# choderalab/pymbar

Measured on AMD Instinct MI355X. Metric: mbar_adaptive_iterations_per_sec, higher is better.
Workload: dtype f64

## Files before the change

### pymbar_amd/csrc/mbar_device.h

```cpp
#ifndef MBAR_DEVICE_H
#define MBAR_DEVICE_H
#include "mbar_internal.h"

#include <hip/hip_ext.h>
#include <math.h>
#include <type_traits>

namespace mbar {

typedef double v4d __attribute__((ext_vector_type(4)));

template <int CTRL>
__device__ __forceinline__ double dpp_move(double x) {
    int lo = __double2loint(x), hi = __double2hiint(x);
    lo = __builtin_amdgcn_update_dpp(0, lo, CTRL, 0xF, 0xF, true);
    hi = __builtin_amdgcn_update_dpp(0, hi, CTRL, 0xF, 0xF, true);
    return __hiloint2double(hi, lo);
}
__device__ __forceinline__ double row16_max(double x) {
    x = fmax(x, dpp_move<0xB1>(x));
    x = fmax(x, dpp_move<0x4E>(x));
    x = fmax(x, dpp_move<0x141>(x));
    x = fmax(x, dpp_move<0x140>(x));
    return x;
}
template <int N>
__device__ __forceinline__ double row16_bcast(double x) {
    double r;
    asm("v_mov_b64_dpp %0, %1 row_newbcast:%2 row_mask:0xf bank_mask:0xf" : "=v"(r) : "v"(x), "n"(N));
    return r;
}
__device__ __forceinline__ double row16_sum(double x) {
    x += dpp_move<0xB1>(x);
    x += dpp_move<0x4E>(x);
    x += dpp_move<0x141>(x);
    x += dpp_move<0x140>(x);
    return x;
}
template <int M>
__device__ __forceinline__ double lane_xor(double x) {
    if constexpr (M >= 16) {
        return __shfl_xor(x, M);
    } else if constexpr (M == 8) {
        return dpp_move<0x128>(x);
    } else if constexpr (M == 4) {
        int lo = __double2loint(x), hi = __double2hiint(x);
        int tl = __builtin_amdgcn_update_dpp(lo, lo, 0x104, 0xF, 0x5, false);
        tl = __builtin_amdgcn_update_dpp(tl, lo, 0x114, 0xF, 0xA, false);
        int th = __builtin_amdgcn_update_dpp(hi, hi, 0x104, 0xF, 0x5, false);
        th = __builtin_amdgcn_update_dpp(th, hi, 0x114, 0xF, 0xA, false);
        return __hiloint2double(th, tl);
    } else if constexpr (M == 2) {
        return dpp_move<0x4E>(x);
    } else {
        return dpp_move<0xB1>(x);
    }
}
__device__ __forceinline__ double wave_sum(double x) {
#pragma unroll
    for (int m = 32; m >= 1; m >>= 1) x += __shfl_xor(x, m);
    return x;
}
__device__ __forceinline__ double wave_max(double x) {
#pragma unroll
    for (int m = 32; m >= 1; m >>= 1) x = fmax(x, __shfl_xor(x, m));
    return x;
}
__device__ __forceinline__ double block256_sum(double v, double* red ) {
    v = wave_sum(v);
    __syncthreads();
    if ((threadIdx.x & 63) == 0) red[threadIdx.x >> 6] = v;
    __syncthreads();
    return (red[0] + red[1]) + (red[2] + red[3]);
}
__device__ __forceinline__ double block256_max(double v, double* red ) {
    v = wave_max(v);
    __syncthreads();
    if ((threadIdx.x & 63) == 0) red[threadIdx.x >> 6] = v;
    __syncthreads();
    return fmax(fmax(red[0], red[1]), fmax(red[2], red[3]));
}

#include "exp2_table.inc"
#include "log_table.inc"
constexpr double LOG2E = 0x1.71547652b82fep+0, LN2 = 0x1.62e42fefa39efp-1;
constexpr double EXP2_S = (double)(1 << EXP2_BITS);
constexpr double LOG2E_S = EXP2_S * LOG2E, LN2_OVER_S = LN2 / EXP2_S;
constexpr double EXP2_CLAMP = -1100.0 * EXP2_S;
constexpr int EXP2_TABLE_BYTES = (1 << EXP2_BITS) * 8;
constexpr int LOG_TABLE_BYTES = 256 * 8;
constexpr int EXP_TABLE_BYTES = EXP2_TABLE_BYTES + LOG_TABLE_BYTES;
constexpr int EXP_TABLE_DMA_PER_WAVE = (EXP_TABLE_BYTES / 1024 + 7) / 8;
typedef __attribute__((address_space(3))) const double lds_cdouble;
__device__ __forceinline__ void exp_table_init(char* smem) {
    if ((uint32_t)(uintptr_t)(__attribute__((address_space(3))) char*)smem != 0u) __builtin_trap();
    for (int i = threadIdx.x; i < (1 << EXP2_BITS); i += blockDim.x) reinterpret_cast<double*>(smem)[i] = EXP2_TABLE[i];
    for (int i = threadIdx.x; i < 256; i += blockDim.x)
        reinterpret_cast<double*>(smem + EXP2_TABLE_BYTES)[i] = LOG_TABLE[i];
}
__device__ __forceinline__ void exp_table_init_dma(char* smem) {
    if ((uint32_t)(uintptr_t)(__attribute__((address_space(3))) char*)smem != 0u) __builtin_trap();
    const int lane = threadIdx.x & 63;
    const int wave = __builtin_amdgcn_readfirstlane(threadIdx.x >> 6), nwv = blockDim.x >> 6;
    constexpr int NCH = EXP_TABLE_BYTES / 1024, NCH_EXP = EXP2_TABLE_BYTES / 1024;
    const int per_wave = (NCH + nwv - 1) / nwv;
    for (int i = 0; i < per_wave; ++i) {
        const int c = (wave + i * nwv) % NCH;
        const char* src = c < NCH_EXP ? reinterpret_cast<const char*>(EXP2_TABLE) + c * 1024
                                      : reinterpret_cast<const char*>(LOG_TABLE) + (c - NCH_EXP) * 1024;
        __builtin_amdgcn_global_load_lds((const __attribute__((address_space(1))) void*)(src + lane * 16),
                                         (__attribute__((address_space(3))) void*)(smem + c * 1024), 16, 0, 0);
    }
}
__device__ __forceinline__ double exp2_table_at(int si) {
    return *(lds_cdouble*)(uintptr_t)(uint32_t)((si << 3) & (EXP2_TABLE_BYTES - 8));
}
__device__ __forceinline__ double exp2_poly(double z) {
    double p = EXP2_POLY[EXP2_DEG];
#pragma unroll
    for (int k = EXP2_DEG - 1; k >= 0; --k) p = fma(p, z, EXP2_POLY[k]);
    return p;
}
__device__ __forceinline__ double exp2s_fast(double ts) {
    const double t = fmax(ts, EXP2_CLAMP);
    const double s = __builtin_rint(t);
    const double z = t - s;
    const int si = (int)s;
    const double T = exp2_table_at(si);
    return ldexp(T * exp2_poly(z), si >> EXP2_BITS);
}
typedef double v2d __attribute__((ext_vector_type(2)));
__device__ __forceinline__ double log_pos(double s) {
    const double m = __builtin_amdgcn_frexp_mant(s);
    const double ed = (double)__builtin_amdgcn_frexp_exp(s);
    const uint32_t off = (uint32_t)(__double2hiint(m) >> 9) & 0x7f0u;
    const v2d tc = *(__attribute__((address_space(3))) const v2d*)(uintptr_t)(uint32_t)(EXP2_TABLE_BYTES + off);
    const double r = fma(m, tc.x, -1.0);
    double q = -1.0 / 6.0;
    q = fma(q, r, 0.2);
    q = fma(q, r, -0.25);
    q = fma(q, r, 1.0 / 3.0);
    q = fma(q, r, -0.5);
    q = fma(q, r, 1.0);
    return fma(ed, LN2, tc.y) + q * r;
}
template <int N, bool CLAMP = true>
__device__ __forceinline__ void exp2s_batch(double (&x)[N]) {
    double T[N];
    int q[N];
#pragma unroll
    for (int i = 0; i < N; ++i) {
        const double t = CLAMP ? fmax(x[i], EXP2_CLAMP) : x[i];
        const double s = __builtin_rint(t);
        x[i] = t - s;
        const int si = (int)s;
        q[i] = si >> EXP2_BITS;
        T[i] = exp2_table_at(si);
    }
    __builtin_amdgcn_sched_barrier(0);
#pragma unroll
    for (int i = 0; i < N; ++i) x[i] = exp2_poly(x[i]);
    __builtin_amdgcn_sched_barrier(0);
#pragma unroll
    for (int i = 0; i < N; ++i) x[i] = ldexp(T[i] * x[i], q[i]);
}
template <int N>
__device__ __forceinline__ void exp2s_batch2(double (&x0)[N], double (&x1)[N]) {
    double T0[N], T1[N];
    int q0[N], q1[N];
#pragma unroll
    for (int i = 0; i < N; ++i) {
        const double t0 = fmax(x0[i], EXP2_CLAMP), t1 = fmax(x1[i], EXP2_CLAMP);
        const double s0 = __builtin_rint(t0), s1 = __builtin_rint(t1);
        x0[i] = t0 - s0;
        x1[i] = t1 - s1;
        const int i0 = (int)s0, i1 = (int)s1;
        q0[i] = i0 >> EXP2_BITS;
        q1[i] = i1 >> EXP2_BITS;
        T0[i] = exp2_table_at(i0);
        T1[i] = exp2_table_at(i1);
    }
    __builtin_amdgcn_sched_barrier(0);
#pragma unroll
    for (int i = 0; i < N; ++i) {
        x0[i] = exp2_poly(x0[i]);
        x1[i] = exp2_poly(x1[i]);
    }
    __builtin_amdgcn_sched_barrier(0);
#pragma unroll
    for (int i = 0; i < N; ++i) {
        x0[i] = ldexp(T0[i] * x0[i], q0[i]);
        x1[i] = ldexp(T1[i] * x1[i], q1[i]);
    }
}
constexpr double EXP2N_POLY[4] = {1.0, -0x1.62e42fefa3028p-12, 0x1.ebfbdf9648000p-25, -0x1.c69cea0000000p-38};
template <int N, bool CLAMP>
__device__ __forceinline__ void exp2s_neg_batch(double (&w)[N]) {
    double T[N];
    int q[N];
#pragma unroll
    for (int i = 0; i < N; ++i) {
        const double t = CLAMP ? fmin(w[i], 2.0e9) : w[i];
        const int ni = (int)(-t);
        w[i] = __builtin_amdgcn_fract(t);
        q[i] = ni >> EXP2_BITS;
        T[i] = exp2_table_at(ni);
    }
    __builtin_amdgcn_sched_barrier(0);
#pragma unroll
    for (int i = 0; i < N; ++i) {
        double p = EXP2N_POLY[3];
        p = fma(p, w[i], EXP2N_POLY[2]);
        p = fma(p, w[i], EXP2N_POLY[1]);
        w[i] = fma(p, w[i], EXP2N_POLY[0]);
    }
    __builtin_amdgcn_sched_barrier(0);
#pragma unroll
    for (int i = 0; i < N; ++i) w[i] = ldexp(T[i] * w[i], q[i]);
}
template <int N, bool CLAMP>
__device__ __forceinline__ void exp2s_neg_batch2(double (&w0)[N], double (&w1)[N]) {
    double T0[N], T1[N];
    int q0[N], q1[N];
#pragma unroll
    for (int i = 0; i < N; ++i) {
        const double t0 = CLAMP ? fmin(w0[i], 2.0e9) : w0[i], t1 = CLAMP ? fmin(w1[i], 2.0e9) : w1[i];
        const int n0 = (int)(-t0), n1 = (int)(-t1);
        w0[i] = __builtin_amdgcn_fract(t0);
        w1[i] = __builtin_amdgcn_fract(t1);
        q0[i] = n0 >> EXP2_BITS;
        q1[i] = n1 >> EXP2_BITS;
        T0[i] = exp2_table_at(n0);
        T1[i] = exp2_table_at(n1);
    }
    __builtin_amdgcn_sched_barrier(0);
#pragma unroll
    for (int i = 0; i < N; ++i) {
        double p0 = EXP2N_POLY[3], p1 = EXP2N_POLY[3];
        p0 = fma(p0, w0[i], EXP2N_POLY[2]);
        p1 = fma(p1, w1[i], EXP2N_POLY[2]);
        p0 = fma(p0, w0[i], EXP2N_POLY[1]);
        p1 = fma(p1, w1[i], EXP2N_POLY[1]);
        w0[i] = fma(p0, w0[i], EXP2N_POLY[0]);
        w1[i] = fma(p1, w1[i], EXP2N_POLY[0]);
    }
    __builtin_amdgcn_sched_barrier(0);
#pragma unroll
    for (int i = 0; i < N; ++i) {
        w0[i] = ldexp(T0[i] * w0[i], q0[i]);
        w1[i] = ldexp(T1[i] * w1[i], q1[i]);
    }
}
__device__ __forceinline__ double recip_fast(double s) {
    double r = __builtin_amdgcn_rcp(s);
    r = fma(fma(-s, r, 1.0), r, r);
    r = fma(fma(-s, r, 1.0), r, r);
    return r;
}

template <int NB>
__device__ __forceinline__ double tree_max(const double (&x)[NB]) {
    double t[NB];
#pragma unroll
    for (int i = 0; i < NB; ++i) t[i] = x[i];
#pragma unroll
    for (int n = NB; n > 1; n -= n / 2) {
#pragma unroll
        for (int i = 0; i < n / 2; ++i) t[i] = fmax(t[i], t[n - 1 - i]);
    }
    return t[0];
}
template <int NB>
__device__ __forceinline__ double tree_sum(const double (&x)[NB]) {
    double t[NB];
#pragma unroll
    for (int i = 0; i < NB; ++i) t[i] = x[i];
#pragma unroll
    for (int n = NB; n > 1; n -= n / 2) {
#pragma unroll
        for (int i = 0; i < n / 2; ++i) t[i] += t[n - 1 - i];
    }
    return t[0];
}
template <int NB>
__device__ __forceinline__ double dot_sum(const double (&x)[NB], const double (&c)[NB]) {
    if constexpr (NB == 1) {
        return x[0] * c[0];
    } else {
        double e = x[0] * c[0], o = x[1] * c[1];
#pragma unroll
        for (int i = 2; i + 1 < NB; i += 2) {
            e = fma(x[i], c[i], e);
            o = fma(x[i + 1], c[i + 1], o);
        }
        if constexpr (NB & 1) e = fma(x[NB - 1], c[NB - 1], e);
        return e + o;
    }
}
__device__ __forceinline__ void row16_max2(double& a, double& b) {
    a = fmax(a, dpp_move<0xB1>(a));   b = fmax(b, dpp_move<0xB1>(b));
    a = fmax(a, dpp_move<0x4E>(a));   b = fmax(b, dpp_move<0x4E>(b));
    a = fmax(a, dpp_move<0x141>(a));  b = fmax(b, dpp_move<0x141>(b));
    a = fmax(a, dpp_move<0x140>(a));  b = fmax(b, dpp_move<0x140>(b));
}
__device__ __forceinline__ void row16_sum2(double& a, double& b) {
    a += dpp_move<0xB1>(a);   b += dpp_move<0xB1>(b);
    a += dpp_move<0x4E>(a);   b += dpp_move<0x4E>(b);
    a += dpp_move<0x141>(a);  b += dpp_move<0x141>(b);
    a += dpp_move<0x140>(a);  b += dpp_move<0x140>(b);
}
template <int NF>
__device__ __forceinline__ void logden_out(double mm, const double (&ss)[NF], int ks, bool sample_ok, int64_t n,
                                           double wn, double* __restrict__ logden0, double* __restrict__ logden1,
                                           const double* __restrict__ dn, double& objl) {
    const bool second = NF == 2 && (ks & 4);
    const double s_first = ss[0], s_second = ss[NF - 1];
    const double ldv = fma(mm, LN2_OVER_S, log_pos(second ? s_second : s_first));
    if (sample_ok && ks < 4 * NF) {
        double* out = second ? logden1 : logden0;
        if (out) out[n] = ldv;
        objl = fma(wn, dn ? (ldv - dn[n]) : ldv, objl);
    }
}
template <int NF>
__device__ __forceinline__ void objective_out(double objl, int ks, int lane, double* __restrict__ obj_part, int64_t rec) {
#pragma unroll
    for (int f = 0; f < NF; ++f) {
        const double o = wave_sum((ks >> 2) == f ? objl : 0.0);
        if (lane == 0) obj_part[rec * NF + f] = o;
    }
}
template <int NB>
__device__ __forceinline__ void lse_load2(const char* cbuf, int rd0, int rd1, const double (&a)[NB],
                                          double (&x0)[NB], double (&x1)[NB]) {
#pragma unroll
    for (int I = 0; I < NB; ++I) {
        x0[I] = *reinterpret_cast<const double*>(cbuf + I * (16 * TS * 8) + rd0);
        x1[I] = *reinterpret_cast<const double*>(cbuf + I * (16 * TS * 8) + rd1);
    }
    __builtin_amdgcn_sched_barrier(0);
#pragma unroll
    for (int I = 0; I < NB; ++I) {
        x0[I] = a[I] - x0[I];
        x1[I] = a[I] - x1[I];
    }
}
template <int NB, int NF, bool SPLIT = false>
__device__ __forceinline__ void lse_math2(double (&x0)[NB], double (&x1)[NB], const double (&c)[NB],
                                          double (&acc)[NF][NB], double w0, double w1, double& m2_0, double& m2_1,
                                          double (&s0)[NF], double (&s1)[NF]) {
    double m0 = tree_max<NB>(x0), m1 = tree_max<NB>(x1);
    row16_max2(m0, m1);
    m2_0 = m0 * LOG2E_S;
    m2_1 = m1 * LOG2E_S;
#pragma unroll
    for (int I = 0; I < NB; ++I) {
        x0[I] = fma(x0[I], LOG2E_S, -m2_0);
        x1[I] = fma(x1[I], LOG2E_S, -m2_1);
    }
    if constexpr (SPLIT) {
        exp2s_batch<NB>(x0);
        exp2s_batch<NB>(x1);
    } else {
        exp2s_batch2<NB>(x0, x1);
    }
#pragma unroll
    for (int f = 0; f < NF; ++f) {
        s0[f] = f == 0 ? tree_sum<NB>(x0) : dot_sum<NB>(x0, c);
        s1[f] = f == 0 ? tree_sum<NB>(x1) : dot_sum<NB>(x1, c);
        row16_sum2(s0[f], s1[f]);
        const double r0 = w0 * recip_fast(s0[f]), r1 = w1 * recip_fast(s1[f]);
#pragma unroll
        for (int I = 0; I < NB; ++I) acc[f][I] = fma(x1[I], r1, fma(x0[I], r0, acc[f][I]));
    }
}
template <int NB, int NF>
__device__ __forceinline__ void lse_two_groups(const char* cbuf, int rd0, int rd1,
                                               const double (&a)[NB], const double (&c)[NB], double (&acc)[NF][NB],
                                               double w0, double w1, double& m2_0, double& m2_1,
                                               double (&s0)[NF], double (&s1)[NF]) {
    double x0[NB], x1[NB];
    lse_load2<NB>(cbuf, rd0, rd1, a, x0, x1);
    lse_math2<NB, NF>(x0, x1, c, acc, w0, w1, m2_0, m2_1, s0, s1);
}

template <int NB>
__device__ __forceinline__ void lse_load1(const char* cbuf, int rd0, const double (&a)[NB], double (&x0)[NB]) {
#pragma unroll
    for (int I = 0; I < NB; ++I) x0[I] = *reinterpret_cast<const double*>(cbuf + I * (16 * TS * 8) + rd0);
    __builtin_amdgcn_sched_barrier(0);
#pragma unroll
    for (int I = 0; I < NB; ++I) x0[I] = a[I] - x0[I];
}
template <int NB, int NF>
__device__ __forceinline__ void lse_math1(double (&x0)[NB], const double (&c)[NB], double (&acc)[NF][NB], double w0,
                                          double& m2_0, double (&s0)[NF]) {
    m2_0 = row16_max(tree_max<NB>(x0)) * LOG2E_S;
#pragma unroll
    for (int I = 0; I < NB; ++I) x0[I] = fma(x0[I], LOG2E_S, -m2_0);
    exp2s_batch<NB>(x0);
#pragma unroll
    for (int f = 0; f < NF; ++f) {
        s0[f] = row16_sum(f == 0 ? tree_sum<NB>(x0) : dot_sum<NB>(x0, c));
        const double r0 = w0 * recip_fast(s0[f]);
#pragma unroll
        for (int I = 0; I < NB; ++I) acc[f][I] = fma(x0[I], r0, acc[f][I]);
    }
}
template <int NB, int NF>
__device__ __forceinline__ void lse_one_group(const char* cbuf, int rd0, const double (&a)[NB],
                                              const double (&c)[NB], double (&acc)[NF][NB], double w0, double& m2_0,
                                              double (&s0)[NF]) {
    double x0[NB];
    lse_load1<NB>(cbuf, rd0, a, x0);
    lse_math1<NB, NF>(x0, c, acc, w0, m2_0, s0);
}
template <int NB, int NF>
__device__ __forceinline__ void lse_group_pair(const char* cbuf, const char* wslot, int rd_base,
                                               const int (&pos)[GROUPS], int g, const double (&a)[NB],
                                               const double (&c)[NB], double (&acc)[NF][NB], int ks, int ns,
                                               double& mm, double (&ss)[NF]) {
    double m2a, m2b, sa[NF], sb[NF];
    const double va = *reinterpret_cast<const double*>(wslot + (4 * g + ns) * 8);
    const double vb = *reinterpret_cast<const double*>(wslot + (4 * (g + 1) + ns) * 8);
    if constexpr (NB <= 8) {
        lse_two_groups<NB, NF>(cbuf, rd_base + pos[g], rd_base + pos[g + 1], a, c, acc, va, vb, m2a, m2b, sa, sb);
    } else {
        lse_one_group<NB, NF>(cbuf, rd_base + pos[g], a, c, acc, va, m2a, sa);
        lse_one_group<NB, NF>(cbuf, rd_base + pos[g + 1], a, c, acc, vb, m2b, sb);
    }
    if ((ks & 3) == g) {
        mm = m2a;
#pragma unroll
        for (int f = 0; f < NF; ++f) ss[f] = sa[f];
    }
    if ((ks & 3) == g + 1) {
        mm = m2b;
#pragma unroll
        for (int f = 0; f < NF; ++f) ss[f] = sb[f];
    }
}

template <bool WIDE>
struct StageOffsetsT {
    typedef typename std::conditional<WIDE, uint64_t, uint32_t>::type off_t;
    off_t off[2];
};
typedef StageOffsetsT<false> StageOffsets;
template <bool WIDE = false>
__device__ __forceinline__ StageOffsetsT<WIDE> make_stage_offsets(int64_t ld, int lane) {
    StageOffsetsT<WIDE> so;
    const int r = lane >> 3, pos = 2 * (lane & 7);
#pragma unroll
    for (int par = 0; par < 2; ++par) {
        const int smp = (pos - ((r & 6) | (par << 3))) & 15;
        so.off[par] = (typename StageOffsetsT<WIDE>::off_t)(((int64_t)r * ld + smp) * 8);
    }
    return so;
}
#ifndef MBAR_DMA_AUX
#define MBAR_DMA_AUX 0
#endif
template <bool DMA>
__device__ __forceinline__ void stage_piece(const double* __restrict__ ubase , uint64_t voff,
                                            char* dst , int lane) {
    const char* src = reinterpret_cast<const char*>(ubase) + voff;
    if constexpr (DMA) {
        __builtin_amdgcn_global_load_lds((const __attribute__((address_space(1))) void*)src,
                                         (__attribute__((address_space(3))) void*)dst, 16, 0, MBAR_DMA_AUX);
    } else {
        *reinterpret_cast<double2*>(dst + lane * 16) = *reinterpret_cast<const double2*>(src);
    }
}
template <bool DMA>
__device__ __forceinline__ void stage_piece(const double* __restrict__ ubase , uint32_t voff,
                                            char* dst , int lane) {
    uint64_t ub = reinterpret_cast<uint64_t>(ubase);
    asm("" : "+s"(ub));
    asm("" : "+v"(voff));
    const char* src = reinterpret_cast<const char*>(ub) + voff;
    if constexpr (DMA) {
        __builtin_amdgcn_global_load_lds((const __attribute__((address_space(1))) void*)src,
                                         (__attribute__((address_space(3))) void*)dst, 16, 0, MBAR_DMA_AUX);
    } else {
        *reinterpret_cast<double2*>(dst + lane * 16) = *reinterpret_cast<const double2*>(src);
    }
}
template <int ROWS, bool DMA, int J0, int JSTEP, typename RowMap, typename SO>
__device__ __forceinline__ void stage_tile(const double* __restrict__ u, int64_t ld, int64_t n0, char* dst, int lane,
                                           const SO& so, RowMap rowmap) {
    constexpr int NDMA = ROWS / 8;
#pragma unroll
    for (int j = J0; j < NDMA; j += JSTEP)
        stage_piece<DMA>(u + rowmap(8 * j) * ld + rowmap.cols(j, n0), so.off[j & 1], dst + j * 1024, lane);
}

template <bool DMA>
__device__ __forceinline__ void stage_vec16(const double* __restrict__ v, int64_t n0, char* dst, int lane) {
    if (lane < 8) stage_piece<DMA>(v + n0, (uint32_t)(lane * 16), dst, lane);
}

__device__ __forceinline__ void settle(double& x) { asm volatile("" : "+v"(x)); }

__device__ __forceinline__ double load_untracked(const double* p) {
    double v;
    asm volatile("global_load_dwordx2 %0, %1, off" : "=v"(v) : "v"(p) : "memory");
    return v;
}
template <int N>
__device__ __forceinline__ void wait_vm_for(double& a, double& b, double& c, double& d, double& e, double (&r)[16]) {
    asm volatile("s_waitcnt vmcnt(%21)"
                 : "+v"(a), "+v"(b), "+v"(c), "+v"(d), "+v"(e), "+v"(r[0]), "+v"(r[1]), "+v"(r[2]), "+v"(r[3]), "+v"(r[4]), "+v"(r[5]),
                   "+v"(r[6]), "+v"(r[7]), "+v"(r[8]), "+v"(r[9]), "+v"(r[10]), "+v"(r[11]), "+v"(r[12]), "+v"(r[13]), "+v"(r[14]), "+v"(r[15])
                 : "n"(N)
                 : "memory");
}
__device__ __forceinline__ void lds_barrier() { asm volatile("s_waitcnt lgkmcnt(0)\n\ts_barrier" ::: "memory"); }
template <int N>
__device__ __forceinline__ void wait_vm() {
    asm volatile("s_waitcnt vmcnt(%0)" ::"n"(N) : "memory");
}

struct RowIdentity {
    int64_t row0;
    uint32_t live = 0xffffffffu;
    __device__ __forceinline__ int64_t operator()(int tr) const { return row0 + tr; }
    __device__ __forceinline__ int64_t cols(int j, int64_t n0) const { return ((live >> j) & 1u) ? n0 : 0; }
};
struct RowTwoPanels {
    int64_t row_i0, row_j0;
    int split;
    uint32_t live = 0xffffffffu;
    __device__ __forceinline__ int64_t operator()(int tr) const {
        return tr < split ? row_i0 + tr : row_j0 + (tr - split);
    }
    __device__ __forceinline__ int64_t cols(int j, int64_t n0) const { return ((live >> j) & 1u) ? n0 : 0; }
};
template <int NB>
__device__ __forceinline__ uint32_t live_piece_mask(const double (&a)[NB], double dead) {
    uint32_t m = 0;
#pragma unroll
    for (int I = 0; I < NB; ++I) {
        const unsigned long long b = __ballot(a[I] != dead);
        m |= ((b & 0xffull) ? 1u : 0u) << (2 * I);
        m |= ((b & 0xff00ull) ? 1u : 0u) << (2 * I + 1);
    }
    return m;
}

constexpr int lse_waves(int nb) { return nb <= 2 ? 16 : (nb <= 4 ? 8 : (nb <= 8 ? 4 : 2)); }
constexpr int TSS = 64;
constexpr int GRAM_AGPR_BLOCKS = 31;
constexpr double GRAM_NEG_HUGE = -2.9e303, LOGDEN_HUGE = 1e300;
constexpr int FUSED_PSUM1_FROM_GRAM_NB = 8;

static inline int blocks_per_cu_for(size_t lds_bytes) {
    int b = (int)((160 * 1024) / lds_bytes);
    if (b < 1) b = 1;
    if (b > 4) b = 4;
    return b;
}

static inline bool stage_offsets_wide(int64_t ld) { return (uint64_t)ld * 56u + 128u >= (1ull << 32); }

hipError_t launch_fused_quad(hipStream_t s, int nbt, const LaunchGeom& g, const double* P, int64_t ld, int64_t N, const double* cmul,
                             const double* cw, const double* wsq, double* rinv0, double* gp, double* pp, const LoopCtl& lc);

__device__ __forceinline__ double family_term(const ScanLinear&, int, double u, double cf, double v, double) { return fma(cf, v, u); }
__device__ __forceinline__ double family_term(const FamilyTerms& terms, int b, double u, double cf, double v, double c) {
#pragma clang fp contract(off)
    if (!((terms.mask >> b) & 1u)) return fma(cf, v, u);
    double dl = v - c;
    const double P = terms.period[b];
    if (P > 0.0) {
        const double m = rint(dl * terms.rperiod[b]);
        dl = fma(-P, m, dl);
    }
    const double q = dl * dl;
    return fma(cf, q, u);
}
__device__ __forceinline__ double family_term(const ScanHarmonic& fam, int b, double u, double cf, double v, double c) {
    return family_term(fam.terms, b, u, cf, v, c);
}
__device__ __forceinline__ double family_center(const ScanLinear&, int, const double (&)[SCAN_MAX_H]) { return 0.0; }
__device__ __forceinline__ double family_center(const ScanHarmonic& fam, int b, const double (&cen)[SCAN_MAX_H]) {
    const int s = __popc(fam.terms.mask & ((1u << b) - 1u));
    const double c0 = cen[0], c1 = cen[1], c2 = cen[2], c3 = cen[3];
    double c = c3;
    c = s == 2 ? c2 : c;
    c = s == 1 ? c1 : c;
    c = s == 0 ? c0 : c;
    return c;
}
__device__ __forceinline__ void family_load_centers(const ScanLinear&, bool, int64_t, double (&cen)[SCAN_MAX_H]) {
#pragma unroll
    for (int h = 0; h < SCAN_MAX_H; ++h) cen[h] = 0.0;
}
__device__ __forceinline__ void family_load_centers(const ScanHarmonic& fam, bool live, int64_t l, double (&cen)[SCAN_MAX_H]) {
#pragma unroll
    for (int h = 0; h < SCAN_MAX_H; ++h) cen[h] = live ? fam.center[l * SCAN_MAX_H + h] : 0.0;
}

template <class Fam>
__device__ __forceinline__ double scan_x(const ScanData& d, const Fam& fam, const double (&cf)[SCAN_MAX_B], const double (&cen)[SCAN_MAX_H],
                                         double off, int64_t n) {
    double u = off;
#pragma unroll
    for (int b = 0; b < SCAN_MAX_B; ++b)
        if (b < d.B) u = family_term(fam, b, u, cf[b], d.basis[(int64_t)b * d.ldv + n], family_center(fam, b, cen));
    return -u - d.logden[n];
}

}
#endif
```

### pymbar_amd/csrc/mbar_k_fused.hip

```cpp
#include "mbar_device.h"

namespace mbar {

template <int NB>
__host__ __device__ constexpr int fused_steps_done(int I) {
    if (I < 0) return 0;
    if (I >= NB - 2) return 2 * NB;
    if (NB < 4) return 2 * (I + 1) < 2 * NB ? 2 * (I + 1) : 2 * NB;
    const int r1 = (NB + 1) / 2 - 1;
    if (I <= r1) return 2 * (I + 1) < NB ? 2 * (I + 1) : NB;
    const int rows = NB - 2 - r1;
    return NB + (NB * (I - r1) + rows - 1) / rows;
}
template <int NB, bool WIDE, bool UNIT>
__global__ void __launch_bounds__(256, 1)
k_fused(const double* __restrict__ P, int64_t ld, int64_t N, int64_t ntiles, const double* __restrict__ cmul,
        const double* __restrict__ cw, const double* __restrict__ wsq, double* __restrict__ rinv0,
        double* __restrict__ rinv1, double* __restrict__ gram_part, double* __restrict__ psum_part,
        const int* __restrict__ ctl, int64_t slot_stride) {
    extern __shared__ __attribute__((aligned(16))) char smem[];
    if (ctl) {
        if (ctl[CTL_DONE] != 0 || ctl[CTL_LIGHT] != 0) return;
        const int s = ctl[CTL_SLOT];
        rinv1 = rinv0 + (int64_t)((s + 2) % 3) * slot_stride;
        rinv0 = rinv0 + (int64_t)((s + 1) % 3) * slot_stride;
    }
    constexpr int ROWS = NB * 16;
    constexpr int NDMA = ROWS / 8 + (UNIT ? 0 : 1);
    constexpr int U_BYTES = ROWS * TS * 8;
    constexpr int TILE_BYTES = U_BYTES + (UNIT ? 0 : 1024);
    constexpr int NBLK = NB * (NB + 1) / 2;
    constexpr bool PINNED = NBLK > GRAM_AGPR_BLOCKS;
    constexpr bool ACC1 = NB < FUSED_PSUM1_FROM_GRAM_NB;
    const int lane = threadIdx.x & 63;
    const int wave = __builtin_amdgcn_readfirstlane(threadIdx.x >> 6);
    const int nwv = blockDim.x >> 6;
    const int ks = lane & 15, ns = lane >> 4;
    char* buf = smem + wave * (2 * TILE_BYTES);
    const int64_t gw = (int64_t)blockIdx.x * nwv + wave;
    const int64_t W = (int64_t)gridDim.x * nwv;
    RowIdentity rows{0};
    const StageOffsetsT<WIDE> so = make_stage_offsets<WIDE>(ld, lane);

    double acc[2][NB];
#pragma unroll
    for (int f = 0; f < 2; ++f)
#pragma unroll
        for (int I = 0; I < NB; ++I) acc[f][I] = 0.0;
    {
        double cany[NB];
#pragma unroll
        for (int I = 0; I < NB; ++I) cany[I] = fabs(cmul[16 * I + ks]) + fabs(cmul[ROWS + 16 * I + ks]);
        if constexpr (NB <= 2) rows.live = live_piece_mask<NB>(cany, 0.0);
    }
    constexpr int NSTEP = ROWS / 4;
    double cb[UNIT ? NSTEP : 1];
    if constexpr (UNIT) {
#pragma unroll
        for (int st = 0; st < NSTEP; ++st) {
            const double cv = cmul[(lane & 1) * ROWS + 4 * st + (lane >> 4)];
            cb[st] = (lane & 3) < 2 ? cv : 0.0;
            asm volatile("" : "+v"(cb[st]));
        }
    } else {
        double* ctab = reinterpret_cast<double*>(smem + nwv * (2 * TILE_BYTES));
        for (int e = threadIdx.x; e < NSTEP * 16; e += blockDim.x) ctab[e] = (e & 3) < 2 ? cmul[(e & 3) * ROWS + (e >> 2)] : 0.0;
        __syncthreads();
    }
    int apos[4];
#pragma unroll
    for (int q = 0; q < 4; ++q) apos[q] = ns * (TS * 8) + (((lane & 15) + (ns & 2) + 4 * q) & 15) * 8;
    v4d G[NBLK];
#pragma unroll
    for (int b = 0; b < NBLK; ++b) G[b] = v4d{0.0, 0.0, 0.0, 0.0};

    const int rd_base = ks * (TS * 8);
    int pos[GROUPS];
#pragma unroll
    for (int g = 0; g < GROUPS; ++g) pos[g] = ((4 * g + ns + (ks & 14)) & 15) * 8;
    const int sq = ns + 4 * ((lane >> 2) & 3);
    const int fq = lane & 3;

    const char* wsrc = reinterpret_cast<const char*>(((lane >> 3) & 1) ? wsq : cw) + (lane & 7) * 16;
    auto stage_w = [&](int64_t tile, char* dst) {
        __builtin_amdgcn_global_load_lds((const __attribute__((address_space(1))) void*)(wsrc + tile * (TS * 8)),
                                         (__attribute__((address_space(3))) void*)(dst + U_BYTES), 16, 0, 0);
    };
    auto stage = [&](int64_t tile, char* dst) {
        stage_tile<ROWS, true, 0, 1>(P, ld, tile * TS, dst, lane, so, rows);
        if constexpr (!UNIT) stage_w(tile, dst);
    };
    auto read_group = [&](const char* tb, int g, double (&x)[NB], double& wg, double& swg) {
        if constexpr (!UNIT) {
            wg = *reinterpret_cast<const double*>(tb + U_BYTES + (4 * g + ns) * 8);
            swg = *reinterpret_cast<const double*>(tb + U_BYTES + TS * 8 + (4 * g + ns) * 8);
        }
#pragma unroll
        for (int I = 0; I < NB; ++I) x[I] = *reinterpret_cast<const double*>(tb + I * (16 * TS * 8) + rd_base + pos[g]);
    };
    uint32_t cop_off = (uint32_t)(nwv * (2 * TILE_BYTES) + (lane >> 4) * 32 + (lane & 3) * 8);
    auto read_step = [&](const char* tb, int st, double& a, double& b) {
        a = *reinterpret_cast<const double*>(tb + st * (4 * TS * 8) + apos[st & 3]);
        if constexpr (UNIT) b = cb[st];
        else b = *reinterpret_cast<const double*>(smem + cop_off + st * 128);
    };
    auto mfma4 = [&](double& d, double a, double b, bool first) {
        if constexpr (PINNED) {
            if (first)
                asm volatile("v_mfma_f64_4x4x4_4b_f64 %0, %1, %2, 0" : "=v"(d) : "v"(a), "v"(b));
            else
                asm volatile("v_mfma_f64_4x4x4_4b_f64 %0, %1, %2, %0" : "+v"(d) : "v"(a), "v"(b));
        } else {
            d = __builtin_amdgcn_mfma_f64_4x4x4f64(a, b, first ? 0.0 : d, 0, 0, 0);
        }
    };
    auto store_rinv = [&](int64_t tile, double& r) {
        const int64_t n = tile * TS + sq;
        double* out = fq ? rinv1 : rinv0;
        if constexpr (UNIT) r = n < N ? r : 0.0;
        if (n < N && fq < 2) out[n] = r;
    };
    int64_t t = gw;
    int cur = 0;
    double rcur = 0.0;
    double uv[2][NB], w[2], sw[2];
    if (t < ntiles) {
        stage(t, buf);
        if (t + W < ntiles) {
            stage(t + W, buf + TILE_BYTES);
            wait_vm<NDMA>();
        } else {
            wait_vm<0>();
        }
        double sa = 0.0, sb = 0.0;
#pragma unroll
        for (int st = 0; st < NSTEP; st += 2) {
            double a0, b0, a1, b1;
            read_step(buf, st, a0, b0);
            read_step(buf, st + 1, a1, b1);
            sa = __builtin_amdgcn_mfma_f64_4x4x4f64(a0, b0, sa, 0, 0, 0);
            sb = __builtin_amdgcn_mfma_f64_4x4x4f64(a1, b1, sb, 0, 0, 0);
        }
        rcur = recip_fast(fmax(sa + sb, 1e-300));
        store_rinv(t, rcur);
        read_group(buf, 0, uv[0], w[0], sw[0]);
    }
    for (; t < ntiles; t += W) {
        char* cbuf = buf + cur * TILE_BYTES;
        char* nbuf = buf + (cur ^ 1) * TILE_BYTES;
        const int64_t tn = t + W, tnn = t + 2 * W;
        const int64_t tstage = tnn < ntiles ? tnn : t;
        if constexpr (!UNIT) asm volatile("" : "+v"(cop_off));
        double sacc[4];
#pragma unroll
        for (int g = 0; g < GROUPS; ++g) {
            const int gc = g & 1, gn = gc ^ 1;
            if (g == 2) wait_vm<1>();
            double r0, r1;
            switch (g) {
                case 0: r0 = row16_bcast<0>(rcur); r1 = row16_bcast<1>(rcur); break;
                case 1: r0 = row16_bcast<4>(rcur); r1 = row16_bcast<5>(rcur); break;
                case 2: r0 = row16_bcast<8>(rcur); r1 = row16_bcast<9>(rcur); break;
                default: r0 = row16_bcast<12>(rcur); r1 = row16_bcast<13>(rcur); break;
            }
            const double q0 = UNIT ? r0 : w[gc] * r0, q1 = UNIT ? r1 : w[gc] * r1;
#pragma unroll
            for (int I = 0; I < NB; ++I) {
                acc[0][I] = fma(uv[gc][I], q0, acc[0][I]);
                if constexpr (ACC1) acc[1][I] = fma(uv[gc][I], q1, acc[1][I]);
                settle(acc[0][I]);
                if constexpr (ACC1) settle(acc[1][I]);
            }
            const double rin = UNIT ? r1 : r1 * sw[gc];
            double p[NB];
#pragma unroll
            for (int I = 0; I < NB; ++I) p[I] = uv[gc][I] * rin;
            constexpr int B1 = NB >= 4 ? NB : 2 * NB;
            double opa[B1], opb[B1];
            auto request_next = [&]() {
                if (g < GROUPS - 1) {
                    read_group(cbuf, g + 1, uv[gn], w[gn], sw[gn]);
                } else {
                    read_group(nbuf, 0, uv[gn], w[gn], sw[gn]);
                }
            };
            auto request_steps = [&]() {
                if (g >= 2) {
#pragma unroll
                    for (int q = 0; q < B1; ++q) read_step(nbuf, (g - 2) * 2 * NB + q, opa[q], opb[q]);
                }
            };
            if constexpr (!PINNED) {
                request_next();
                request_steps();
            }
            auto mfma = [&](int b, double x, double y) {
                if constexpr (PINNED) {
                    if (b < GRAM_AGPR_BLOCKS)
                        asm volatile("v_mfma_f64_16x16x4_f64 %0, %1, %2, %0" : "+a"(G[b]) : "v"(x), "v"(y));
                    else
                        asm volatile("v_mfma_f64_16x16x4_f64 %0, %1, %2, %0" : "+v"(G[b]) : "v"(x), "v"(y));
                } else {
                    G[b] = __builtin_amdgcn_mfma_f64_16x16x4f64(x, y, G[b], 0, 0, 0);
                }
            };
            if constexpr (PINNED) {
                __builtin_amdgcn_sched_barrier(0);
                asm volatile("s_nop 7");
            }
            constexpr int NM = NBLK;
            int b = 0, nm = 0;
#pragma unroll
            for (int I = 0; I < NB; ++I) {
                if (NB == 1 && g >= 2) {
                    mfma4(sacc[2 * (g & 1)], opa[0], opb[0], true);
                    mfma4(sacc[2 * (g & 1) + 1], opa[1], opb[1], true);
                }
#pragma unroll
                for (int J = I; J < NB; ++J) {
                    mfma(b, p[I], p[J]);
                    if constexpr (PINNED) {
                        if (nm == 0 || nm == 1) {
                            __builtin_amdgcn_sched_barrier(0);
                            if (nm == 0) request_next(); else request_steps();
                            __builtin_amdgcn_sched_barrier(0);
                        }
                    }
                    if (g == GROUPS - 1) {
#pragma unroll
                        for (int j = nm * NDMA / NM; j < (nm + 1) * NDMA / NM; ++j) {
                            if constexpr (PINNED) __builtin_amdgcn_sched_barrier(0);
                            if (j < ROWS / 8)
                                stage_piece<true>(P + rows(8 * j) * ld + rows.cols(j, tstage * TS), so.off[j & 1], cbuf + j * 1024, lane);
                            else if constexpr (!UNIT)
                                stage_w(tstage, cbuf);
                            if constexpr (PINNED) __builtin_amdgcn_sched_barrier(0);
                        }
                    }
                    ++b;
                    ++nm;
                }
                if (g >= 2 && NB > 1 && I < NB - 1) {
#pragma unroll
                    for (int q = fused_steps_done<NB>(I - 1); q < fused_steps_done<NB>(I); ++q)
                        mfma4(sacc[q & 3], opa[q % B1], opb[q % B1], g == 2 && q < 4);
                    if (B1 < 2 * NB && fused_steps_done<NB>(I - 1) < B1 && fused_steps_done<NB>(I) >= B1) {
#pragma unroll
                        for (int q = 0; q < B1; ++q) read_step(nbuf, (g - 2) * 2 * NB + B1 + q, opa[q], opb[q]);
                    }
                }
            }
            if constexpr (PINNED) __builtin_amdgcn_sched_barrier(0);
        }
        if constexpr (PINNED)
            asm volatile("s_nop 7\n\ts_nop 7" : "+v"(sacc[0]), "+v"(sacc[1]), "+v"(sacc[2]), "+v"(sacc[3]));
        rcur = recip_fast(fmax((sacc[0] + sacc[1]) + (sacc[2] + sacc[3]), 1e-300));
        store_rinv(tn, rcur);
        cur ^= 1;
    }
    if constexpr (PINNED) asm volatile("s_nop 15\n\ts_nop 15" ::: "memory");
#pragma unroll
    for (int f = 0; f < 2; ++f) {
#pragma unroll
        for (int I = 0; I < NB; ++I) {
            double v = acc[f][I];
            v += __shfl_xor(v, 16);
            v += __shfl_xor(v, 32);
            if (lane < 16) psum_part[(gw * 2 + f) * ROWS + 16 * I + lane] = v;
        }
    }
    {
        int b = 0;
#pragma unroll
        for (int I = 0; I < NB; ++I)
#pragma unroll
            for (int J = I; J < NB; ++J, ++b) {
#pragma unroll
                for (int r = 0; r < 4; ++r) {
#if defined(MBAR_GRAM_STORE_NT)
                    __builtin_nontemporal_store(G[b][r], &gram_part[((gw * NBLK + b) * 4 + r) * 64 + lane]);
#else
                    gram_part[((gw * NBLK + b) * 4 + r) * 64 + lane] = G[b][r];
#endif
                }
            }
    }
}



LaunchGeom fused_geometry(int nb, int num_cu, int64_t ntiles, int64_t grid_override, bool unit) {
    LaunchGeom g;
    g.waves = 4;
    g.variant = 1;
    if (nb > 8) {
        g.variant = 6;
        g.lds_bytes = (size_t)2 * ((size_t)nb * 16 * TS * 8 + 4 * 1024) + 1024;
        int64_t capq = grid_override > 0 ? grid_override : num_cu;
        int64_t wantq = ntiles < 1 ? 1 : ntiles;
        g.blocks = (int)(wantq < capq ? wantq : capq);
        g.nwaves = g.blocks;
        g.psum_records = g.nwaves;
        return g;
    }
    const size_t tile = (size_t)nb * 16 * TS * 8 + 1024;
    const size_t lds_general = (size_t)4 * 2 * tile + (size_t)nb * 512;
    g.lds_bytes = unit ? (size_t)4 * 2 * (tile - 1024) : lds_general;
    int64_t want = (ntiles + 3) / 4;
    int64_t cap = num_cu;
    if (nb <= 5) {
        static const int occ[6] = {1, 4, 4, 3, 2, 2};
        const int by_lds = blocks_per_cu_for(lds_general);
        cap = (int64_t)num_cu * (by_lds < occ[nb] ? by_lds : occ[nb]);
        int64_t by_work = (ntiles + 127) / 128;
        if (by_work < num_cu) by_work = num_cu;
        if (cap > by_work) cap = by_work;
    }
    if (grid_override > 0) cap = grid_override;
    if (want < 1) want = 1;
    g.blocks = (int)(want < cap ? want : cap);
    g.nwaves = g.blocks * 4;
    g.psum_records = g.nwaves;
    return g;
}
template <int NB>
static hipError_t launch_fused_nb(hipStream_t s, const LaunchGeom& g, const double* P, int64_t ld, int64_t N, const double* cmul,
                                  const double* cw, const double* wsq, bool unit, double* rinv0, double* gp, double* pp, const LoopCtl& lc) {
    auto go = [&](auto kern) -> hipError_t {
        if (g.lds_bytes > 64 * 1024) {
            hipError_t e = hipFuncSetAttribute(reinterpret_cast<const void*>(kern),
                                               hipFuncAttributeMaxDynamicSharedMemorySize, (int)g.lds_bytes);
            if (e != hipSuccess) return e;
        }
        const int64_t ntiles = (N + TS - 1) / TS;
        double* r1 = nullptr;
        if (lc.ev_start && lc.ev_stop)
            hipExtLaunchKernelGGL(kern, dim3(g.blocks), dim3(256), g.lds_bytes, s, lc.ev_start, lc.ev_stop, 0, P, ld, N, ntiles, cmul,
                                  cw, wsq, rinv0, r1, gp, pp, lc.ctl, lc.slot_stride);
        else
            hipLaunchKernelGGL(kern, dim3(g.blocks), dim3(256), g.lds_bytes, s, P, ld, N, ntiles, cmul, cw, wsq, rinv0, r1, gp, pp,
                               lc.ctl, lc.slot_stride);
        return hipGetLastError();
    };
    if (unit) return stage_offsets_wide(ld) ? go(k_fused<NB, true, true>) : go(k_fused<NB, false, true>);
    return stage_offsets_wide(ld) ? go(k_fused<NB, true, false>) : go(k_fused<NB, false, false>);
}
hipError_t launch_fused(hipStream_t s, int nb, const LaunchGeom& g, const double* P, int64_t ld, int64_t N, const double* cmul,
                        const double* cw, const double* wsq, bool unit, double* rinv_base, double* gram_part, double* psum_part,
                        const LoopCtl& lc) {
    if (!lc.ctl) return hipErrorInvalidValue;
    if (nb == 12 || nb == 16) return launch_fused_quad(s, nb, g, P, ld, N, cmul, cw, wsq, rinv_base, gram_part, psum_part, lc);
    switch (nb) {
#define MBAR_CASE(NB_) \
    case NB_: return launch_fused_nb<NB_>(s, g, P, ld, N, cmul, cw, wsq, unit, rinv_base, gram_part, psum_part, lc);
        MBAR_CASE(1) MBAR_CASE(2) MBAR_CASE(3) MBAR_CASE(4) MBAR_CASE(5) MBAR_CASE(6) MBAR_CASE(7) MBAR_CASE(8)
#undef MBAR_CASE
        default: return hipErrorInvalidValue;
    }
}

}
```

Before: 297.3.

## Cut address and broadcast overhead in fused tile loop of MBAR kernel

Reworks the fused kernel's inner loop to reduce scalar and vector instruction overhead. LDS addresses are precomputed as 32-bit absolute offsets, and the double-buffer index becomes a compile-time constant by unrolling the tile loop in pairs. The reciprocal-inverse store now uses exec-masked inline assembly with a precomputed base and a ballot. In the unit-weight path, a DPP broadcast is fused into v_fmac_f64_dpp. Global piece addresses are built incrementally by pitch, and the launcher falls back to the wide offset path for very large slot strides. The cost is considerably more inline asm and index logic, which adds correctness risk.

```diff
diff --git a/pymbar_amd/csrc/mbar_device.h b/pymbar_amd/csrc/mbar_device.h
--- a/pymbar_amd/csrc/mbar_device.h
+++ b/pymbar_amd/csrc/mbar_device.h
@@ -29,6 +29,10 @@
     double r;
     asm("v_mov_b64_dpp %0, %1 row_newbcast:%2 row_mask:0xf bank_mask:0xf" : "=v"(r) : "v"(x), "n"(N));
     return r;
+}
+template <int N>
+__device__ __forceinline__ void fmac_row16_bcast(double& acc, double r, double x) {
+    asm("v_fmac_f64_dpp %0, %1, %2 row_newbcast:%3 row_mask:0xf bank_mask:0xf" : "+v"(acc) : "v"(r), "v"(x), "n"(N));
 }
 __device__ __forceinline__ double row16_sum(double x) {
     x += dpp_move<0xB1>(x);
diff --git a/pymbar_amd/csrc/mbar_k_fused.hip b/pymbar_amd/csrc/mbar_k_fused.hip
--- a/pymbar_amd/csrc/mbar_k_fused.hip
+++ b/pymbar_amd/csrc/mbar_k_fused.hip
@@ -40,7 +40,7 @@
     const int64_t gw = (int64_t)blockIdx.x * nwv + wave;
     const int64_t W = (int64_t)gridDim.x * nwv;
     RowIdentity rows{0};
-    const StageOffsetsT<WIDE> so = make_stage_offsets<WIDE>(ld, lane);
+    StageOffsetsT<WIDE> so = make_stage_offsets<WIDE>(ld, lane);
 
     double acc[2][NB];
 #pragma unroll
@@ -67,19 +67,34 @@
         for (int e = threadIdx.x; e < NSTEP * 16; e += blockDim.x) ctab[e] = (e & 3) < 2 ? cmul[(e & 3) * ROWS + (e >> 2)] : 0.0;
         __syncthreads();
     }
-    int apos[4];
-#pragma unroll
-    for (int q = 0; q < 4; ++q) apos[q] = ns * (TS * 8) + (((lane & 15) + (ns & 2) + 4 * q) & 15) * 8;
+    const uint32_t bufo = (uint32_t)(uintptr_t)(__attribute__((address_space(3))) char*)buf;
+    uint32_t apos[4];
+#pragma unroll
+    for (int q = 0; q < 4; ++q) {
+        apos[q] = bufo + ns * (TS * 8) + (((lane & 15) + (ns & 2) + 4 * q) & 15) * 8;
+        asm volatile("" : "+v"(apos[q]));
+    }
     v4d G[NBLK];
 #pragma unroll
     for (int b = 0; b < NBLK; ++b) G[b] = v4d{0.0, 0.0, 0.0, 0.0};
 
-    const int rd_base = ks * (TS * 8);
-    int pos[GROUPS];
-#pragma unroll
-    for (int g = 0; g < GROUPS; ++g) pos[g] = ((4 * g + ns + (ks & 14)) & 15) * 8;
+    uint32_t pos[GROUPS];
+#pragma unroll
+    for (int g = 0; g < GROUPS; ++g) {
+        pos[g] = bufo + ks * (TS * 8) + ((4 * g + ns + (ks & 14)) & 15) * 8;
+        asm volatile("" : "+v"(pos[g]));
+    }
+    [[maybe_unused]] uint32_t wpos = bufo + U_BYTES + ns * 8;
+    if constexpr (!UNIT) asm volatile("" : "+v"(wpos));
     const int sq = ns + 4 * ((lane >> 2) & 3);
     const int fq = lane & 3;
+    const bool up1 = reinterpret_cast<uintptr_t>(rinv1) > reinterpret_cast<uintptr_t>(rinv0);
+    char* const rlo = reinterpret_cast<char*>(up1 ? rinv0 : rinv1);
+    const uint64_t rgap = up1 ? reinterpret_cast<uintptr_t>(rinv1) - reinterpret_cast<uintptr_t>(rinv0)
+                              : reinterpret_cast<uintptr_t>(rinv0) - reinterpret_cast<uintptr_t>(rinv1);
+    typename StageOffsetsT<WIDE>::off_t roff = (typename StageOffsetsT<WIDE>::off_t)(((fq == 1) == up1 ? rgap : 0) + sq * 8);
+    const int sqs = fq < 2 ? sq : TS;
+    const int nlast = (int)(N - (ntiles - 1) * TS);
 
     const char* wsrc = reinterpret_cast<const char*>(((lane >> 3) & 1) ? wsq : cw) + (lane & 7) * 16;
     auto stage_w = [&](int64_t tile, char* dst) {
@@ -90,17 +105,18 @@
         stage_tile<ROWS, true, 0, 1>(P, ld, tile * TS, dst, lane, so, rows);
         if constexpr (!UNIT) stage_w(tile, dst);
     };
-    auto read_group = [&](const char* tb, int g, double (&x)[NB], double& wg, double& swg) {
+    auto lds_at = [](uint32_t a) { return *(lds_cdouble*)(uintptr_t)a; };
+    auto read_group = [&](int tb, int g, double (&x)[NB], double& wg, double& swg) {
         if constexpr (!UNIT) {
-            wg = *reinterpret_cast<const double*>(tb + U_BYTES + (4 * g + ns) * 8);
-            swg = *reinterpret_cast<const double*>(tb + U_BYTES + TS * 8 + (4 * g + ns) * 8);
-        }
-#pragma unroll
-        for (int I = 0; I < NB; ++I) x[I] = *reinterpret_cast<const double*>(tb + I * (16 * TS * 8) + rd_base + pos[g]);
+            wg = lds_at(wpos + (tb + 4 * g * 8));
+            swg = lds_at(wpos + (tb + TS * 8 + 4 * g * 8));
+        }
+#pragma unroll
+        for (int I = 0; I < NB; ++I) x[I] = lds_at(pos[g] + (tb + I * (16 * TS * 8)));
     };
     uint32_t cop_off = (uint32_t)(nwv * (2 * TILE_BYTES) + (lane >> 4) * 32 + (lane & 3) * 8);
-    auto read_step = [&](const char* tb, int st, double& a, double& b) {
-        a = *reinterpret_cast<const double*>(tb + st * (4 * TS * 8) + apos[st & 3]);
+    auto read_step = [&](int tb, int st, double& a, double& b) {
+        a = lds_at(apos[st & 3] + (tb + st * (4 * TS * 8)));
         if constexpr (UNIT) b = cb[st];
         else b = *reinterpret_cast<const double*>(smem + cop_off + st * 128);
     };
@@ -114,20 +130,50 @@
             d = __builtin_amdgcn_mfma_f64_4x4x4f64(a, b, first ? 0.0 : d, 0, 0, 0);
         }
     };
-    auto store_rinv = [&](int64_t tile, double& r) {
-        const int64_t n = tile * TS + sq;
-        double* out = fq ? rinv1 : rinv0;
-        if constexpr (UNIT) r = n < N ? r : 0.0;
-        if (n < N && fq < 2) out[n] = r;
+    auto store_rinv = [&](int64_t tile, int nv, double& r) {
+        const bool ok = sqs < nv;
+        if constexpr (UNIT) r = ok ? r : 0.0;
+        const uint64_t okm = __builtin_amdgcn_ballot_w64(ok);
+        const uint64_t sb = reinterpret_cast<uint64_t>(rlo + tile * (TS * 8));
+        uint64_t saved;
+        if constexpr (WIDE) {
+            const uint64_t a = sb + roff;
+            asm volatile("s_and_saveexec_b64 %0, %2\n\tglobal_store_dwordx2 %3, %1, off\n\ts_mov_b64 exec, %0"
+                         : "=&s"(saved), "+v"(r) : "s"(okm), "v"(a) : "memory", "scc");
+        } else {
+            asm volatile("s_and_saveexec_b64 %0, %2\n\tglobal_store_dwordx2 %3, %1, %4\n\ts_mov_b64 exec, %0"
+                         : "=&s"(saved), "+v"(r) : "s"(okm), "v"(roff), "s"(sb) : "memory", "scc");
+        }
+    };
+    const uint64_t pitch8 = (uint64_t)ld * 64;
+    auto request_piece = [&](int j, int64_t tile, char* dst, uint64_t& ub) {
+        if constexpr (NB <= 2)
+            ub = reinterpret_cast<uint64_t>(P + rows(8 * j) * ld + rows.cols(j, tile * TS));
+        else
+            ub = j == 0 ? reinterpret_cast<uint64_t>(P + tile * TS) : ub + pitch8;
+        if constexpr (WIDE) {
+            asm("" : "+s"(ub));
+            stage_piece<true>(reinterpret_cast<const double*>(ub), so.off[j & 1], dst, lane);
+        } else {
+            asm("" : "+s"(ub));
+            asm("" : "+v"(so.off[j & 1]));
+            __builtin_amdgcn_global_load_lds((const __attribute__((address_space(1))) void*)(reinterpret_cast<const char*>(ub) + so.off[j & 1]),
+                                             (__attribute__((address_space(3))) void*)dst, 16, 0, MBAR_DMA_AUX);
+        }
     };
     int64_t t = gw;
-    int cur = 0;
+    const int Wn = (int)W;
+    int left = (int)(ntiles - gw);
+    auto count_of = [&](int l) { return l > 1 ? TS : (l == 1 ? nlast : 0); };
     double rcur = 0.0;
     double uv[2][NB], w[2], sw[2];
-    if (t < ntiles) {
-        stage(t, buf);
-        if (t + W < ntiles) {
-            stage(t + W, buf + TILE_BYTES);
+    int first = 0;
+    if (left > 0) {
+        first = (int)(((uint32_t)(left - 1) / (uint32_t)Wn + 1u) & 1u);
+        const int fb = first * TILE_BYTES;
+        stage(t, buf + fb);
+        if (left > Wn) {
+            stage(t + W, buf + (TILE_BYTES - fb));
             wait_vm<NDMA>();
         } else {
             wait_vm<0>();
@@ -136,37 +182,47 @@
 #pragma unroll
         for (int st = 0; st < NSTEP; st += 2) {
             double a0, b0, a1, b1;
-            read_step(buf, st, a0, b0);
-            read_step(buf, st + 1, a1, b1);
+            read_step(fb, st, a0, b0);
+            read_step(fb, st + 1, a1, b1);
             sa = __builtin_amdgcn_mfma_f64_4x4x4f64(a0, b0, sa, 0, 0, 0);
             sb = __builtin_amdgcn_mfma_f64_4x4x4f64(a1, b1, sb, 0, 0, 0);
         }
         rcur = recip_fast(fmax(sa + sb, 1e-300));
-        store_rinv(t, rcur);
-        read_group(buf, 0, uv[0], w[0], sw[0]);
-    }
-    for (; t < ntiles; t += W) {
-        char* cbuf = buf + cur * TILE_BYTES;
-        char* nbuf = buf + (cur ^ 1) * TILE_BYTES;
+        store_rinv(t, count_of(left), rcur);
+        read_group(fb, 0, uv[0], w[0], sw[0]);
+    }
+    auto tile_step = [&](const int CUR) __attribute__((always_inline)) {
+        const int CB = CUR * TILE_BYTES, NXB = (CUR ^ 1) * TILE_BYTES;
+        char* cbuf = buf + CB;
         const int64_t tn = t + W, tnn = t + 2 * W;
-        const int64_t tstage = tnn < ntiles ? tnn : t;
+        const int64_t tstage = left > 2 * Wn ? tnn : t;
+        uint64_t piece_src = 0;
         if constexpr (!UNIT) asm volatile("" : "+v"(cop_off));
         double sacc[4];
-#pragma unroll
-        for (int g = 0; g < GROUPS; ++g) {
+        [[maybe_unused]] double r1n = 0.0;
+        auto group_step = [&](const int g) __attribute__((always_inline)) {
             const int gc = g & 1, gn = gc ^ 1;
             if (g == 2) wait_vm<1>();
-            double r0, r1;
+            double r0 = 0.0, r1;
             switch (g) {
-                case 0: r0 = row16_bcast<0>(rcur); r1 = row16_bcast<1>(rcur); break;
-                case 1: r0 = row16_bcast<4>(rcur); r1 = row16_bcast<5>(rcur); break;
-                case 2: r0 = row16_bcast<8>(rcur); r1 = row16_bcast<9>(rcur); break;
-                default: r0 = row16_bcast<12>(rcur); r1 = row16_bcast<13>(rcur); break;
+                case 0: if constexpr (!UNIT) r0 = row16_bcast<0>(rcur); r1 = row16_bcast<1>(rcur); break;
+                case 1: if constexpr (!UNIT) { r0 = row16_bcast<4>(rcur); r1 = row16_bcast<5>(rcur); } else { r1 = r1n; } break;
+                case 2: if constexpr (!UNIT) { r0 = row16_bcast<8>(rcur); r1 = row16_bcast<9>(rcur); } else { r1 = r1n; } break;
+                default: if constexpr (!UNIT) { r0 = row16_bcast<12>(rcur); r1 = row16_bcast<13>(rcur); } else { r1 = r1n; } break;
             }
             const double q0 = UNIT ? r0 : w[gc] * r0, q1 = UNIT ? r1 : w[gc] * r1;
 #pragma unroll
             for (int I = 0; I < NB; ++I) {
-                acc[0][I] = fma(uv[gc][I], q0, acc[0][I]);
+                if constexpr (UNIT) {
+                    switch (g) {
+                        case 0: fmac_row16_bcast<0>(acc[0][I], rcur, uv[gc][I]); break;
+                        case 1: fmac_row16_bcast<4>(acc[0][I], rcur, uv[gc][I]); break;
+                        case 2: fmac_row16_bcast<8>(acc[0][I], rcur, uv[gc][I]); break;
+                        default: fmac_row16_bcast<12>(acc[0][I], rcur, uv[gc][I]); break;
+                    }
+                } else {
+                    acc[0][I] = fma(uv[gc][I], q0, acc[0][I]);
+                }
                 if constexpr (ACC1) acc[1][I] = fma(uv[gc][I], q1, acc[1][I]);
                 settle(acc[0][I]);
                 if constexpr (ACC1) settle(acc[1][I]);
@@ -175,19 +231,27 @@
             double p[NB];
 #pragma unroll
             for (int I = 0; I < NB; ++I) p[I] = uv[gc][I] * rin;
+            if constexpr (UNIT) {
+                switch (g) {
+                    case 0: r1n = row16_bcast<5>(rcur); break;
+                    case 1: r1n = row16_bcast<9>(rcur); break;
+                    case 2: r1n = row16_bcast<13>(rcur); break;
+                    default: break;
+                }
+            }
             constexpr int B1 = NB >= 4 ? NB : 2 * NB;
             double opa[B1], opb[B1];
             auto request_next = [&]() {
                 if (g < GROUPS - 1) {
-                    read_group(cbuf, g + 1, uv[gn], w[gn], sw[gn]);
+                    read_group(CB, g + 1, uv[gn], w[gn], sw[gn]);
                 } else {
-                    read_group(nbuf, 0, uv[gn], w[gn], sw[gn]);
+                    read_group(NXB, 0, uv[gn], w[gn], sw[gn]);
                 }
             };
             auto request_steps = [&]() {
                 if (g >= 2) {
 #pragma unroll
-                    for (int q = 0; q < B1; ++q) read_step(nbuf, (g - 2) * 2 * NB + q, opa[q], opb[q]);
+                    for (int q = 0; q < B1; ++q) read_step(NXB, (g - 2) * 2 * NB + q, opa[q], opb[q]);
                 }
             };
             if constexpr (!PINNED) {
@@ -231,7 +295,7 @@
                         for (int j = nm * NDMA / NM; j < (nm + 1) * NDMA / NM; ++j) {
                             if constexpr (PINNED) __builtin_amdgcn_sched_barrier(0);
                             if (j < ROWS / 8)
-                                stage_piece<true>(P + rows(8 * j) * ld + rows.cols(j, tstage * TS), so.off[j & 1], cbuf + j * 1024, lane);
+                                request_piece(j, tstage, cbuf + j * 1024, piece_src);
                             else if constexpr (!UNIT)
                                 stage_w(tstage, cbuf);
                             if constexpr (PINNED) __builtin_amdgcn_sched_barrier(0);
@@ -246,17 +310,30 @@
                         mfma4(sacc[q & 3], opa[q % B1], opb[q % B1], g == 2 && q < 4);
                     if (B1 < 2 * NB && fused_steps_done<NB>(I - 1) < B1 && fused_steps_done<NB>(I) >= B1) {
 #pragma unroll
-                        for (int q = 0; q < B1; ++q) read_step(nbuf, (g - 2) * 2 * NB + B1 + q, opa[q], opb[q]);
+                        for (int q = 0; q < B1; ++q) read_step(NXB, (g - 2) * 2 * NB + B1 + q, opa[q], opb[q]);
                     }
                 }
             }
             if constexpr (PINNED) __builtin_amdgcn_sched_barrier(0);
-        }
+        };
+        static_assert(GROUPS == 4, "the tile loop names its four groups");
+        group_step(0);
+        group_step(1);
+        group_step(2);
+        group_step(3);
         if constexpr (PINNED)
             asm volatile("s_nop 7\n\ts_nop 7" : "+v"(sacc[0]), "+v"(sacc[1]), "+v"(sacc[2]), "+v"(sacc[3]));
         rcur = recip_fast(fmax((sacc[0] + sacc[1]) + (sacc[2] + sacc[3]), 1e-300));
-        store_rinv(tn, rcur);
-        cur ^= 1;
+        store_rinv(tn, count_of(left - Wn), rcur);
+        t = tn;
+        left -= Wn;
+    };
+    int skip = first;
+    while (left > 0) {
+        asm volatile("" : "+s"(skip));
+        if (!skip) tile_step(0);
+        skip = 0;
+        tile_step(1);
     }
     if constexpr (PINNED) asm volatile("s_nop 15\n\ts_nop 15" ::: "memory");
 #pragma unroll
@@ -333,6 +410,7 @@
             if (e != hipSuccess) return e;
         }
         const int64_t ntiles = (N + TS - 1) / TS;
+        if (ntiles > INT32_MAX) return hipErrorInvalidValue;
         double* r1 = nullptr;
         if (lc.ev_start && lc.ev_stop)
             hipExtLaunchKernelGGL(kern, dim3(g.blocks), dim3(256), g.lds_bytes, s, lc.ev_start, lc.ev_stop, 0, P, ld, N, ntiles, cmul,
@@ -342,8 +420,9 @@
                                lc.ctl, lc.slot_stride);
         return hipGetLastError();
     };
-    if (unit) return stage_offsets_wide(ld) ? go(k_fused<NB, true, true>) : go(k_fused<NB, false, true>);
-    return stage_offsets_wide(ld) ? go(k_fused<NB, true, false>) : go(k_fused<NB, false, false>);
+    const bool wide = stage_offsets_wide(ld) || (uint64_t)lc.slot_stride * 16u + 128u >= (1ull << 32);
+    if (unit) return wide ? go(k_fused<NB, true, true>) : go(k_fused<NB, false, true>);
+    return wide ? go(k_fused<NB, true, false>) : go(k_fused<NB, false, false>);
 }
 hipError_t launch_fused(hipStream_t s, int nb, const LaunchGeom& g, const double* P, int64_t ld, int64_t N, const double* cmul,
                         const double* cw, const double* wsq, bool unit, double* rinv_base, double* gram_part, double* psum_part,
```

Measured after the change: 304.5, median of 6. 1.02x the previous value.
